# xerial/genome-weaver-align

Hardware: AMD Instinct MI355X
Metric: reads/sec (whole node), 100 bp k≤2 vs hg19, at 1/2/4/8 MI355X (higher is better)
Workload: dtype u64

## Files before the change

genome-weaver-align_amd/csrc/batch_io.hip:

```cpp
#include <hip/hip_runtime.h>

#include <rocprim/device/device_radix_sort.hpp>
#include <rocprim/device/device_scan.hpp>

#include <cstdlib>
#include <stdexcept>
#include <string>

#include "kernels.h"
#include "sam_core.h"
#include "text_core.h"

namespace gwa {

#define FCHK(x)                                                                                         \
  do {                                                                                                  \
    hipError_t e_ = (x);                                                                                \
    if (e_ != hipSuccess) throw std::runtime_error(std::string("sam_format: ") + #x + ": " + hipGetErrorString(e_)); \
  } while (0)


__device__ __forceinline__ uint8_t to3bitDev(unsigned char c) {
  switch (c) {
    case 'A': case 'a': return 0;
// ... 29 lines not shown
    w[i] = r ? (lo >> r) | (hi << (32 - r)) : lo;
  }
}
__global__ void __launch_bounds__(256) encodeLenKernel(const char *__restrict__ seq, const uint64_t *__restrict__ seqB,
                                                       const uint64_t *__restrict__ seqE, uint32_t n, uint32_t *__restrict__ codeLen,
                                                       uint32_t *__restrict__ rowLen, uint32_t *__restrict__ lenSeen) {
  const uint32_t r = blockIdx.x * blockDim.x + threadIdx.x;
  if (r > n) return;
  if (r == n) {
    rowLen[n] = 16;
    return;
  }
  const uint64_t b = seqB[r], e = seqE[r];
  uint32_t spaces = 0;
  for (uint64_t a = b & ~(uint64_t)15; a < e; a += 16) {
    const u32x4 c = loadChunk(seq, a);
    const uint32_t w[4] = {c.x, c.y, c.z, c.w};
#pragma unroll
    for (int i = 0; i < 4; ++i) {
      const uint64_t p = a + 4 * i;
      uint32_t m = bytesEq(w[i], ' ');
      const int64_t lo = (int64_t)b - (int64_t)p, hi = (int64_t)e - (int64_t)p;
      const uint32_t keepLo = lo <= 0 ? 0xFFFFFFFFu : lo >= 4 ? 0u : (0xFFFFFFFFu << (8 * lo));
      const uint32_t keepHi = hi >= 4 ? 0xFFFFFFFFu : hi <= 0 ? 0u : (0xFFFFFFFFu >> (8 * (4 - hi)));
      spaces += __builtin_popcount(m & keepLo & keepHi);
    }
  }
  const uint32_t m = (uint32_t)(e - b) - spaces;
  codeLen[r] = m;
  rowLen[r] = (m + 15) & ~15u;
  lenSeen[m < kLenSeen - 1 ? m : kLenSeen - 1] = 1;
}

__global__ void __launch_bounds__(256) encodeWriteKernel(const char *__restrict__ seq, const uint64_t *__restrict__ seqB,
                                                         const uint64_t *__restrict__ seqE, uint32_t n,
                                                         const uint32_t *__restrict__ codeOff,
                                                         const uint32_t *__restrict__ codeLen,
                                                         uint8_t *__restrict__ codes) {
  const uint32_t r = blockIdx.x * blockDim.x + threadIdx.x;
  if (r >= n) return;
  uint8_t *o = codes + codeOff[r];
  const uint64_t b = seqB[r], e = seqE[r];
  const uint32_t m = codeLen[r], row = codeOff[r + 1] - codeOff[r];
  if (m == e - b) {
    for (uint32_t k = 0; k < row; k += 16) {
      uint32_t w[4];
      load16(seq, b + k, w);
      u32x4 v;
      uint32_t c[4];
#pragma unroll
      for (int i = 0; i < 4; ++i) {
        const int valid = (int)m - (int)(k + 4 * i);
        const uint32_t keep = valid >= 4 ? 0xFFFFFFFFu : valid <= 0 ? 0u : (0xFFFFFFFFu >> (8 * (4 - valid)));
        c[i] = to3bit4(w[i]) & keep;
      }
      v.x = c[0]; v.y = c[1]; v.z = c[2]; v.w = c[3];
      *reinterpret_cast<u32x4 *>(o + k) = v;
    }
    return;
  }
  uint32_t k = 0;
  for (uint64_t i = b; i < e; ++i)
    if (seq[i] != ' ') o[k++] = to3bitDev((unsigned char)seq[i]);
  for (; k < row; ++k) o[k] = 0;
}

void launchEncode(const char *seq, const uint64_t *seqB, const uint64_t *seqE, uint32_t n, uint32_t *codeLen, uint32_t *rowLen,
                  uint32_t *codeOff, uint32_t *lenSeen, uint8_t *codes, void *scanTmp, size_t scanTmpBytes, int pass,
                  hipStream_t s) {
  const dim3 grid((n + 1 + 255) / 256);
  if (pass == 0) {
    hipLaunchKernelGGL(encodeLenKernel, grid, dim3(256), 0, s, seq, seqB, seqE, n, codeLen, rowLen, lenSeen);
    FCHK(hipGetLastError());
    size_t b = scanTmpBytes;
    FCHK(rocprim::exclusive_scan(scanTmp, b, rowLen, codeOff, (uint32_t)0, (size_t)n + 1, rocprim::plus<uint32_t>(), s));
  } else {
    hipLaunchKernelGGL(encodeWriteKernel, grid, dim3(256), 0, s, seq, seqB, seqE, n, codeOff, codeLen, codes);
    FCHK(hipGetLastError());
  }
}

size_t encodeScanTempBytes(uint32_t n) {
  size_t b = 0;
  FCHK(rocprim::exclusive_scan(nullptr, b, (uint32_t *)nullptr, (uint32_t *)nullptr, (uint32_t)0, (size_t)n + 1,
                               rocprim::plus<uint32_t>(), (hipStream_t)0));
  return b;
}

__device__ __forceinline__ bool isWsDev(unsigned char c) { return c == ' ' || (c >= '\t' && c <= '\r') || (c >= 0x1c && c <= 0x1f); }

__device__ __forceinline__ uint64_t lineAt(const char *__restrict__ t, uint64_t len, uint64_t pos, uint64_t *e) {
  if (pos >= len) {
    *e = len;
    return len;
  }
  uint64_t i = pos;
  while (i < len && t[i] != '\n' && t[i] != '\r') ++i;
  *e = i;
  if (i == len) return len;
  if (t[i] == '\r' && i + 1 < len && t[i + 1] == '\n') return i + 2;
  return i + 1;
}

__global__ void __launch_bounds__(256) fastqFieldsKernel(const char *__restrict__ t, uint64_t len, const uint64_t *__restrict__ start,
                                                         uint32_t n, uint64_t *__restrict__ f, uint32_t *__restrict__ err) {
  const uint32_t r = blockIdx.x * blockDim.x + threadIdx.x;
  if (r >= n) return;
  uint64_t he, se, pe, qe;
  const uint64_t hb = start[r];
  const uint64_t sb = lineAt(t, len, hb, &he);
// ... 16 lines not shown
void launchFastqFields(const char *text, uint64_t len, const uint64_t *start, uint32_t n, uint64_t *fields,
                       uint32_t *err, hipStream_t s) {
  if (n == 0) return;
  hipLaunchKernelGGL(fastqFieldsKernel, dim3((n + 255) / 256), dim3(256), 0, s, text, len, start, n, fields, err);
  FCHK(hipGetLastError());
}


__device__ __forceinline__ int samUnit(SamOut &o, const SamText &t, uint32_t r, const OutHeader *oh, const OutHit *hits,
                                       const uint16_t *cig, const PairSpec &ps) {
  if (ps.np) return samPair(o, t, r, ps.np, oh, hits, cig, ps.minIns, ps.maxIns, ps.resc);
  return samRead(o, t, r, oh[r], hits, cig);
}

__global__ void __launch_bounds__(256) samLenKernel(SamText t, const OutHeader *__restrict__ oh, const OutHit *__restrict__ hits,
                                                    const uint16_t *__restrict__ cig, const uint32_t *__restrict__ idx,
                                                    uint32_t first, uint32_t n, uint64_t *__restrict__ len,
                                                    uint32_t *__restrict__ err, PairSpec ps) {
  const uint32_t j = blockIdx.x * blockDim.x + threadIdx.x;
  if (j > n) return;
  if (j == n) {
    len[n] = 0;
    return;
  }
  const uint32_t r = idx ? idx[j] : first + j;
  SamOut o{nullptr, 0};
  if (samUnit(o, t, r, oh, hits, cig, ps) != 0) {
    atomicMin(err, j);
    o.n = 0;
  }
  len[j] = o.n;
}

template <int STAGE>
__global__ void __launch_bounds__(64) samWriteKernel(SamText t, const OutHeader *__restrict__ oh, const OutHit *__restrict__ hits,
                                                     const uint16_t *__restrict__ cig, const uint32_t *__restrict__ idx,
                                                     uint32_t first, uint32_t n, const uint64_t *__restrict__ off,
                                                     char *__restrict__ out, PairSpec ps) {
  __shared__ u32x4 stage[STAGE / 16];
  const uint32_t j0 = blockIdx.x * 64, j = j0 + threadIdx.x;
  const uint32_t jEnd = j0 + 64 < n ? j0 + 64 : n;
  const uint64_t gBeg = off[j0], gEnd = off[jEnd];
  const uint64_t base = gBeg & ~(uint64_t)15;
  if (gEnd - base > (uint64_t)STAGE) {
    if (j < n) {
      SamOut o{out + off[j], 0};
      (void)samUnit(o, t, idx ? idx[j] : first + j, oh, hits, cig, ps);
    }
    return;
  }
  if (j < n) {
    SamOut o{reinterpret_cast<char *>(stage) + (off[j] - base), 0};
    (void)samUnit(o, t, idx ? idx[j] : first + j, oh, hits, cig, ps);
  }
  __syncthreads();
  const uint32_t chunks = (uint32_t)((gEnd - base + 15) >> 4);
  for (uint32_t c = threadIdx.x; c < chunks; c += 64) {
    const uint64_t a = base + 16ull * c;
    if (a >= gBeg && a + 16 <= gEnd) {
      *reinterpret_cast<u32x4 *>(out + a) = stage[c];
    } else {
      const char *sb = reinterpret_cast<const char *>(stage) + 16ull * c;
      for (int i = 0; i < 16; ++i)
        if (a + i >= gBeg && a + i < gEnd) out[a + i] = sb[i];
    }
  }
}

void launchSamFormat(const SamText &t, const OutHeader *oh, const OutHit *hits, const uint16_t *cig, const uint32_t *idx,
                     uint32_t first, uint32_t n, uint64_t *len, uint64_t *off, void *scanTmp, size_t *scanTmpBytes,
                     uint32_t *err, char *out, int pass, hipStream_t s, const PairSpec &ps, uint64_t totalBytes) {
  const dim3 grid((n + 1 + 255) / 256);
  if (pass == 0) {
    hipLaunchKernelGGL(samLenKernel, grid, dim3(256), 0, s, t, oh, hits, cig, idx, first, n, len, err, ps);
    FCHK(hipGetLastError());
  } else if (pass == 1) {
    FCHK(rocprim::exclusive_scan(scanTmp, *scanTmpBytes, len, off, (uint64_t)0, (size_t)n + 1, rocprim::plus<uint64_t>(), s));
  } else {
    if (n == 0) return;
    const dim3 g64((n + 63) / 64);
    const uint64_t need = n ? totalBytes * 64 * 103 / 100 / n + 16 : 0;
    const char *stg = getenv("GWA_SAM_STAGE");
    if (stg && atoi(stg) > 0) {
      if (atoi(stg) <= 1024)
        hipLaunchKernelGGL(samWriteKernel<1024>, g64, dim3(64), 0, s, t, oh, hits, cig, idx, first, n, off, out, ps);
      else
        hipLaunchKernelGGL(samWriteKernel<4096>, g64, dim3(64), 0, s, t, oh, hits, cig, idx, first, n, off, out, ps);
    } else if (ps.np || need > 32768)
      hipLaunchKernelGGL(samWriteKernel<49152>, g64, dim3(64), 0, s, t, oh, hits, cig, idx, first, n, off, out, ps);
    else if (need > 24576)
      hipLaunchKernelGGL(samWriteKernel<32768>, g64, dim3(64), 0, s, t, oh, hits, cig, idx, first, n, off, out, ps);
    else if (need > 20480 || totalBytes == 0)
      hipLaunchKernelGGL(samWriteKernel<24576>, g64, dim3(64), 0, s, t, oh, hits, cig, idx, first, n, off, out, ps);
    else
      hipLaunchKernelGGL(samWriteKernel<20480>, g64, dim3(64), 0, s, t, oh, hits, cig, idx, first, n, off, out, ps);
    FCHK(hipGetLastError());
  }
}

size_t samScanTempBytes(uint32_t n) {
  size_t b = 0;
  FCHK(rocprim::exclusive_scan(nullptr, b, (uint64_t *)nullptr, (uint64_t *)nullptr, (uint64_t)0, (size_t)n + 1,
                               rocprim::plus<uint64_t>(), (hipStream_t)0));
  return b;
}

__global__ void __launch_bounds__(256) statsKernel(const OutHeader *__restrict__ oh, uint32_t n,
                                                   unsigned long long *__restrict__ acc) {
  __shared__ unsigned long long sh[kStatFields];
  if (threadIdx.x < kStatFields) sh[threadIdx.x] = 0;
  __syncthreads();
  unsigned long long v[kStatFields];
  for (int f = 0; f < kStatFields; ++f) v[f] = 0;
  for (uint32_t r = blockIdx.x * blockDim.x + threadIdx.x; r < n; r += gridDim.x * blockDim.x) {
    const OutHeader &h = oh[r];
    v[0] += (unsigned)h.fmSearches;
    v[1] += (unsigned)h.quickSteps;
    v[2] += (unsigned)h.blocks;
    v[3] += (unsigned)h.searchBlocks;
    v[4] += (unsigned)h.kmerLookups;
    v[5] += (unsigned)h.saReads;
    v[6] += (unsigned)h.quickSa;
    v[7] += (unsigned)h.quickShort;
    v[8] += (unsigned)h.searchShort;
    v[9] += (unsigned)h.states;
    v[10] += (unsigned)h.numSW;
    v[11] += (unsigned)h.verifyBytes;
    v[12] += h.status == ST_MAPPED;
// ... 48 lines not shown
```

genome-weaver-align_amd/csrc/gwa_api.cpp:

```cpp
#include "../../include/gwa.h"

#include <hip/hip_runtime.h>

#include <algorithm>
#include <atomic>
#include <cstdio>
#include <cstdlib>
#include <cstring>
#include <fstream>
#include <map>
#include <mutex>
#include <stdexcept>
#include <string>
#include <thread>
#include <unordered_map>
#include <vector>

#include "bsf_core.h"
#include "sf_core.h"
#include "host_index.h"
#include "kernels.h"
#include "sam.h"
#include "sam_core.h"

// ... 217 lines not shown
  }
  ~Scratch() {
    if (!p) return;
    (void)hipStreamSynchronize(s);
    std::lock_guard<std::mutex> g(ix->scratchMu);
    ix->scratchFree.push_back({p, bytes});
  }
};
}

struct gwa_batch {
  gwa_index *ix = nullptr;
  hipStream_t stream = nullptr;
  gwa_config_t cfg{};
  SearchConfig scfg{};
  uint32_t n = 0;
  bool hasQual = false;
  int maxM = 0, kmax = 0, R = 4;
  bool sfWrap = false;
  char *d_seqText = nullptr, *d_nameText = nullptr, *d_qualText = nullptr;
  const uint64_t *d_seqB = nullptr, *d_seqE = nullptr, *d_nameB = nullptr, *d_nameE = nullptr;
  const uint64_t *d_qualB = nullptr, *d_qualE = nullptr;
  uint8_t *d_qualNull = nullptr;
  uint64_t *d_fieldOwn[3] = {nullptr, nullptr, nullptr};
  uint64_t *d_fmtLen = nullptr, *d_fmtOff = nullptr;
  uint32_t *d_fmtIdx = nullptr, *d_fmtErr = nullptr;
  void *d_fmtTmp = nullptr;
  char *d_fmtText = nullptr;
  size_t fmtCap = 0, fmtTmpBytes = 0, fmtTextCap = 0;
  uint64_t fmtBytes = 0;
  bool fmtWhole = false;
  unsigned long long *d_stats = nullptr;
  bool statsDone = false;
  uint32_t *d_row = nullptr, *d_seen = nullptr;
  void *d_encTmp = nullptr;
  size_t encTmpBytes = 0;
  uint8_t *d_codes = nullptr;
  uint32_t *d_off = nullptr, *d_len = nullptr;
  ScanRes *d_sres = nullptr;
  OutHeader *d_oh = nullptr;
  OutHit *d_hits = nullptr;
  uint16_t *d_cig = nullptr;
  uint32_t *d_list[2] = {nullptr, nullptr};
  uint32_t *d_all = nullptr;
  uint32_t *d_count = nullptr;
  uint64_t *d_stair = nullptr;
  uint32_t *d_stairBase = nullptr;
  uint64_t *d_stairBad = nullptr;
  uint32_t hitCap = 4, cigCap = 64;
  uint64_t poolHits = 0, poolCig = 0;
  uint64_t poolUsedH = 0, poolUsedC = 0;
  StairTables st{};
  gwa_batch_stats_t stats{};
  bool ran = false;
  bool headerOnly = false;
  uint32_t pairs = 0;
  int32_t minIns = 0, maxIns = 0;
  RescueOut *d_rescue = nullptr;
  uint32_t *d_heavy = nullptr;
  std::vector<std::pair<uint32_t, int>> deep;
};

static void freeIndexDev(gwa_index *ix) {
  for (int s = 0; s < 2; ++s) {
    if (ix->d_occ[s]) (void)hipFree(ix->d_occ[s]);
    if (ix->d_sa[s]) (void)hipFree(ix->d_sa[s]);
// ... 359 lines not shown
  }
  SearchConfig &sc = b->scfg;
  sc.k = cfg->k; sc.reportType = cfg->report_type; sc.topL = cfg->top_l; sc.numSplit = cfg->num_split;
  sc.matchScore = cfg->match; sc.mismatchPenalty = cfg->mismatch; sc.splitOpenPenalty = cfg->split_open;
  sc.indelEndSkip = cfg->indel_end_skip; sc.bandWidth = cfg->band_width;
  sc.waitQ16 = getenv("GWA_WAITQ16") ? atoi(getenv("GWA_WAITQ16")) : 0;
  sc.refillMin = 1;
  sc.textSearch = (cfg->num_split <= 1 && !getenv("GWA_NO_TEXT")) ? 1 : 0;
  sc.runAheadMax = getenv("GWA_RUNAHEAD") ? atoi(getenv("GWA_RUNAHEAD")) : 4;
  sc.textCache = getenv("GWA_TEXT_CACHE") ? atoi(getenv("GWA_TEXT_CACHE")) : 0;
  b->stream = batchStream();
  return false;
}

static void batchTail(gwa_batch *b, uint64_t seqBytes) {
  const uint32_t n = b->n;
  const gwa_config_t *cfg = &b->cfg;
  hipStream_t s = b->stream;
  const uint64_t codeBound = seqBytes + 16ull * n + 32;
  if (codeBound > 0xFFFFFFFFull) throw std::runtime_error("read batch too large (> 4 GiB of codes): use fewer reads per batch");
  b->d_codes = bAlloc<uint8_t>(codeBound);
  b->d_off = bAlloc<uint32_t>((size_t)n + 1);
  b->d_len = bAlloc<uint32_t>((size_t)n + 1);
  b->d_row = bAlloc<uint32_t>((size_t)n + 1);
  b->d_seen = bAlloc<uint32_t>(kLenSeen);
  b->encTmpBytes = encodeScanTempBytes(n);
  b->d_encTmp = bAlloc<uint8_t>(b->encTmpBytes);
  std::vector<uint32_t> seen(kLenSeen);
  HIPCHK(hipMemsetAsync(b->d_seen, 0, kLenSeen * sizeof(uint32_t), s));
  launchEncode(b->d_seqText, b->d_seqB, b->d_seqE, n, b->d_len, b->d_row, b->d_off, b->d_seen, b->d_codes, b->d_encTmp,
               b->encTmpBytes, 0, s);
  HIPCHK(hipMemcpyAsync(seen.data(), b->d_seen, kLenSeen * sizeof(uint32_t), hipMemcpyDeviceToHost, s));
  HIPCHK(hipStreamSynchronize(s));
  std::vector<int> lens;
  for (uint32_t m = 0; m < kLenSeen; ++m)
    if (seen[m]) {
      b->maxM = (int)m;
      if ((int)m <= kMaxReadLen) lens.push_back((int)m);
    }
  if (b->maxM > kMaxReadLen)
    throw std::runtime_error("read longer than " + std::to_string(kMaxReadLen) + " bp in this batch (" +
                             std::to_string(b->maxM) + " bp): the device path aligns reads of at most " +
                             std::to_string(kMaxReadLen) + " bp");
  b->sfWrap = false;
  for (int m : lens) {
    int k = (cfg->k > 0 && cfg->k < 1) ? (int)floor((double)((float)m * cfg->k)) : (int)cfg->k;
    b->kmax = std::max(b->kmax, k);
    if (m > 0 && k >= 0 && k <= 31 && sfChunksWrap(m, k + 1)) b->sfWrap = true;
  }
  if (b->kmax > 31) throw std::runtime_error("k > 31 is not supported on the device path");
  {
    const bool sfPath = cfg->strategy == 1;
    const int64_t s = sfPath ? 0 : std::max(1, cfg->num_split), T = (s + 1) * s / 2;
    const int64_t M = std::llabs((int64_t)cfg->match), Nn = std::llabs((int64_t)cfg->mismatch);
    const int64_t S = std::llabs((int64_t)cfg->split_open);
    const int64_t bound = M * b->maxM + (M + Nn) * (255 * (s + 1) + T) + S * T;
    const int lim = sfPath ? 31 : 23;
    if ((!sfPath && cfg->num_split > 64) || bound >= (1LL << lim))
      throw std::runtime_error("scoring parameters too large for the device's queue keys (|score| may reach " +
                               std::to_string(bound) + ", limit 2^" + std::to_string(lim) + ")");
  }
  b->R = b->kmax + 1 <= 4 ? 4 : b->kmax + 1 <= 8 ? 8 : b->kmax + 1 <= 16 ? 16 : 32;
  if (b->scfg.waitQ16 <= 0) b->scfg.waitQ16 = b->R >= 8 ? 8 : 14;
  std::vector<uint64_t> tab, bad;
  std::vector<uint32_t> base;
  buildStairTables(lens, std::max(b->kmax, 0), tab, base, bad);
// ... 224 lines not shown
  hipEvent_t e[3] = {nullptr, nullptr, nullptr};
  Events() {
    for (auto &x : e) HIPCHK(hipEventCreate(&x));
  }
  ~Events() {
    for (auto &x : e)
      if (x) (void)hipEventDestroy(x);
  }
};
}

static SamText samText(const gwa_batch *b);

static int qwFor(int m) { return m <= 128 ? 4 : m <= 256 ? 8 : 16; }

int gwa_batch_run(gwa_batch_t *b) {
  try {
    gwa_index *ix = b->ix;
    HIPCHK(hipSetDevice(ix->device));
    hipStream_t s = b->stream;
    memset(&b->stats, 0, sizeof(b->stats));
    if (b->headerOnly) {
      b->ran = true;
      return 0;
    }
    b->ran = b->statsDone = false;
    b->poolUsedH = b->poolUsedC = 0;
    b->deep.clear();
    ReadsView rv{b->d_codes, b->d_off, b->d_len, b->n};
    Scratch scr(ix, s);
    Events ev;
    hipEvent_t e0 = ev.e[0], e1 = ev.e[1], e2 = ev.e[2];
    HIPCHK(hipEventRecord(e2, s));
    launchEncode(b->d_seqText, b->d_seqB, b->d_seqE, b->n, b->d_len, b->d_row, b->d_off, b->d_seen, b->d_codes,
                 b->d_encTmp, b->encTmpBytes, 0, s);
    launchEncode(b->d_seqText, b->d_seqB, b->d_seqE, b->n, b->d_len, b->d_row, b->d_off, b->d_seen, b->d_codes,
                 b->d_encTmp, b->encTmpBytes, 1, s);
    HIPCHK(hipMemsetAsync(b->d_count, 0, 16 * sizeof(uint32_t), s));
    HIPCHK(hipEventRecord(e0, s));
    const bool sf = b->cfg.strategy == 1;
    if (!sf)
      launchQuickscan(qwFor(b->maxM), ix->view, b->scfg, rv, b->d_sres, b->d_oh, outSlots(b), b->d_list[0],
                      b->d_count, s);
    const bool sfSort = sf && b->R >= 8 && !(getenv("GWA_SEARCH_SORT") && atoi(getenv("GWA_SEARCH_SORT")) == 0);
    if (sfSort) launchKeyscan(qwFor(b->maxM), ix->view, b->scfg, rv, b->d_sres, s);
    HIPCHK(hipGetLastError());
    HIPCHK(hipEventRecord(e1, s));
    uint32_t nSearch = b->n;
    if (!sf) HIPCHK(hipMemcpyAsync(&nSearch, b->d_count, 4, hipMemcpyDeviceToHost, s));
    HIPCHK(hipStreamSynchronize(s));
    float qms = 0, ems = 0;
    HIPCHK(hipEventElapsedTime(&qms, e0, e1));
    HIPCHK(hipEventElapsedTime(&ems, e2, e0));
    b->stats.quickscan_ms = qms;
    b->stats.encode_ms = ems;
    double searchMs = 0;
    int cur = 0;
    uint32_t n = nSearch;
    const bool sortLists = !(getenv("GWA_SEARCH_SORT") && atoi(getenv("GWA_SEARCH_SORT")) == 0);
    bool sfSorted = false;
    const int m = std::max(b->maxM, 1);
    int t = 0, regrow = 0, launches = 0;
    int gArena = 0, gHits = 0, gList = 0, gCigar = 0, gCand = 0;
    int arenaMaxLog = 24;
    if (const char *e = getenv("GWA_MAX_STATES_LOG2"))
      arenaMaxLog = std::max(16, std::min(24, atoi(e)));
    const bool hybrid = !sf && b->R >= 8;
    struct ResBuf {
// ... 773 lines not shown
```

genome-weaver-align_amd/csrc/sam_core.h:

```cpp
#pragma once
#include "gwa_layout.h"

namespace gwa {

struct SamText {
  const char *name;
  const uint64_t *nameB, *nameE;
  const char *qual;
  const uint64_t *qualB, *qualE;
  const uint8_t *qualNull;
  const uint8_t *codes;
  const uint32_t *codeOff, *codeLen;
  const char *ctg;
  const uint64_t *ctgOff;
  const int32_t *chrKey;
  int32_t starKey, emptyKey;
};

struct SamOut {
  char *p;
  uint64_t n;
  GWA_HD void ch(char c) {
    if (p) p[n] = c;
    ++n;
  }
  GWA_HD void bytes(const char *s, uint64_t len) {
    if (p) {
      for (uint64_t i = 0; i < len; i += 16) {
        char b[16];
#pragma unroll
        for (int k = 0; k < 16; ++k) b[k] = i + k < len ? s[i + k] : 0;
#pragma unroll
        for (int k = 0; k < 16; ++k)
          if (i + k < len) p[n + i + k] = b[k];
      }
    }
    n += len;
  }
  template <unsigned long L>
  GWA_HD void lit(const char (&s)[L]) {
    bytes(s, L - 1);
  }
  GWA_HD void num(int64_t v) {
    const bool neg = v < 0;
    uint64_t u = neg ? (uint64_t)(-(v + 1)) + 1 : (uint64_t)v;
    uint64_t d0 = 0, d1 = 0, d2 = 0;
    int k = 0;
    do {
      const uint64_t q = u / 10, dig = u - q * 10;
      if (k < 8) d0 |= dig << (8 * k);
      else if (k < 16) d1 |= dig << (8 * (k - 8));
      else d2 |= dig << (8 * (k - 16));
      ++k;
      u = q;
    } while (u);
    if (neg) ch('-');
    for (int i = k - 1; i >= 0; --i) {
      const uint64_t w = i < 8 ? d0 : i < 16 ? d1 : d2;
      ch((char)('0' + (int)((w >> (8 * (i & 7))) & 0xFF)));
    }
  }
};

GWA_HD bool qualAbsent(const SamText &t, uint32_t r) { return t.qual == nullptr || (t.qualNull && t.qualNull[r]); }

namespace samfmt {

constexpr char kSym[5] = {'A', 'C', 'G', 'T', 'N'};
GWA_HD char sym(unsigned x) { return (char)((0x4E54474341ULL >> (8 * x)) & 0xFF); }
constexpr char kOp[8] = {'M', 'I', 'D', 'N', 'S', 'H', 'P', 'X'};

GWA_HD char stateCh(int numHits) { return numHits > 0 ? (numHits == 1 ? 'U' : 'R') : 'N'; }

struct CigSpec {
  const uint16_t *a;
  int na;
  int preS;
  int postS;
  const uint16_t *b;
  int nb;
};

struct CigEmit {
  SamOut &o;
  int pt = -1;
  int64_t pl = 0;
  GWA_HD explicit CigEmit(SamOut &o_) : o(o_) {}
  GWA_HD void flush() {
    if (pt >= 0) {
      o.num(pl);
      o.ch(kOp[pt & 7]);
    }
  }
  GWA_HD void raw(int t, int64_t l) {
    flush();
    pt = t;
    pl = l;
  }
  GWA_HD void add(int t, int64_t l) {
    if (pt == t) pl += l;
    else raw(t, l);
  }
};
// ... 12 lines not shown
  CigSpec cig;
  int seqA, seqB;
  int qualA, qualB;
  int stateHead, stateSelf;
  bool hasSplit;
};

struct Ctx {
  const SamText &t;
  uint32_t r;
  const OutHit *hits;
  int m;
  int strand;
  bool qualNull;
  uint64_t q0, qn;
  bool npe = false;
};

GWA_HD int32_t nameKey(const Ctx &cx, int chr) {
  if (chr >= 0) return cx.t.chrKey[chr];
  if (chr == CHR_STAR) return cx.t.starKey;
  if (chr == CHR_EMPTY) return cx.t.emptyKey;
  return -2147483647 - 1;
}

GWA_HD void chrName(SamOut &o, Ctx &cx, int chr) {
  if (chr >= 0) o.bytes(cx.t.ctg + cx.t.ctgOff[chr], cx.t.ctgOff[chr + 1] - cx.t.ctgOff[chr]);
  else if (chr == CHR_STAR) o.ch('*');
  else if (chr == CHR_EMPTY) {
  } else cx.npe = true;
}

GWA_HD void emitSeq(SamOut &o, const Ctx &cx, int a, int b) {
  const uint8_t *c = cx.t.codes + cx.t.codeOff[cx.r];
  for (int j0 = a; j0 < b; j0 += 16) {
    uint8_t x[16];
#pragma unroll
    for (int k = 0; k < 16; ++k) {
      const int j = j0 + k;
      x[k] = j < b ? (cx.strand == 0 ? c[j] : c[cx.m - 1 - j]) : 0;
    }
#pragma unroll
    for (int k = 0; k < 16; ++k)
      if (j0 + k < b) o.ch(sym(cx.strand == 0 ? x[k] : (x[k] < 4 ? 3 - x[k] : 4)));
  }
}

GWA_HD void emitQual(SamOut &o, const Ctx &cx, int a, int b) {
  if (cx.qualNull) {
    o.ch('*');
    return;
  }
  const char *q = cx.t.qual + cx.q0;
  for (int j0 = a; j0 < b; j0 += 16) {
    char x[16];
#pragma unroll
    for (int k = 0; k < 16; ++k) {
      const int j = j0 + k;
      x[k] = j < b ? (cx.strand == 0 ? q[j] : q[cx.qn - 1 - j]) : 0;
    }
#pragma unroll
    for (int k = 0; k < 16; ++k)
      if (j0 + k < b) o.ch(x[k]);
  }
}

GWA_HD void emitState(SamOut &o, const Ctx &cx, int head, int self) {
  for (int t = head; t >= 0; t = cx.hits[t].next) {
    const char c = stateCh(cx.hits[t].numHits);
    o.ch(t == self ? c : (char)(c - 'A' + 'a'));
  }
}

GWA_HD bool lineOne(SamOut &o, Ctx &cx, const Rec &r, const Rec *split, bool hasSegments, bool isFirst, bool eachMapped) {
  int flag = 0;
  if (hasSegments) flag |= 0x1;
  if (r.strand == 1) flag |= 0x10;
  if (isFirst) {
    flag |= 0x40;
    if (r.numBestHits <= 0 || (split && split->numBestHits <= 0)) eachMapped = false;
  } else if (!split) {
    flag |= 0x80;
  }
  if (eachMapped) flag |= 0x2;
  if (r.numBestHits <= 0) flag |= 0x4;
  if (split && split->numBestHits <= 0) flag |= 0x8;
  o.bytes(cx.t.name + cx.t.nameB[cx.r], cx.t.nameE[cx.r] - cx.t.nameB[cx.r]);
  o.ch('\t');
  o.num(flag);
  o.ch('\t');
  chrName(o, cx, r.chr);
  o.ch('\t');
  o.num(r.start);
  o.lit("\t1\t");
  emitCigar(o, r.cig);
  if (!split) {
    o.lit("\t*\t0\t0");
  } else {
    const int32_t ck = nameKey(cx, r.chr), sk = nameKey(cx, split->chr);
    if (r.chr != CHR_NULL && split->chr != CHR_NULL && ck != cx.t.starKey && ck == sk) {
      o.lit("\t=");
    } else {
      o.ch('\t');
      chrName(o, cx, split->chr);
    }
    o.ch('\t');
    o.num(split->start);
    o.ch('\t');
    o.num((int64_t)split->end - r.start);
  }
  o.ch('\t');
  emitSeq(o, cx, r.seqA, r.seqB);
  o.ch('\t');
  emitQual(o, cx, r.qualA, r.qualB);
  if (r.numBestHits > 0) {
    if (r.nm >= 0) {
      o.lit("\tNM:i:");
      o.num(r.nm);
    }
    o.lit("\tXP:Z:");
// ... 64 lines not shown
          rec.cig.postS = s.matchLength;
          rec.chr = h.chr; rec.strand = h.strand; rec.start = h.pos; rec.end = h.pos + m; rec.nm = h.diff;
          rec.numBestHits = numHits;
          emitRec(o, cx, rec, nullptr, false);
        } else {
          if (s.chr == CHR_NULL) return -1;
          rec.cig.b = cig + s.cigarOff;
          rec.cig.nb = (int)s.cigarLen;
          rec.chr = s.chr; rec.strand = s.strand; rec.start = s.pos - h.matchLength; rec.end = s.pos - h.matchLength + m;
          rec.nm = s.diff; rec.numBestHits = numHits; rec.stateSelf = h.next;
          emitRec(o, cx, rec, nullptr, false);
        }
      } else {
        if (h.chr == CHR_NULL) return -1;
        rec.cig.postS = s.qEnd - s.qStart;
        rec.chr = h.chr; rec.strand = h.strand; rec.start = h.pos; rec.end = h.pos; rec.nm = h.diff;
        rec.numBestHits = numHits;
        emitRec(o, cx, rec, nullptr, false);
      }
    } else {
      if (!sU) return 0;
      if (s.chr == CHR_NULL) return -1;
      rec.cig = CigSpec{nullptr, 0, h.matchLength, -1, cig + s.cigarOff, (int)s.cigarLen};
      rec.chr = s.chr; rec.strand = s.strand; rec.start = s.pos - h.matchLength; rec.end = s.pos - h.matchLength + m;
      rec.nm = s.diff; rec.numBestHits = numHits; rec.stateSelf = h.next;
      emitRec(o, cx, rec, nullptr, false);
    }
  }
  o.ch('\n');
  return cx.npe ? -1 : 0;
}

GWA_HD void samUnmapped(SamOut &o, const SamText &t, uint32_t r) {
  o.bytes(t.name + t.nameB[r], t.nameE[r] - t.nameB[r]);
  o.lit("\t68\t*\t0\t1\t\t*\t0\t0\t");
  const uint8_t *c = t.codes + t.codeOff[r];
  const uint32_t len = t.codeLen[r];
  for (uint32_t j0 = 0; j0 < len; j0 += 16) {
    uint8_t x[16];
#pragma unroll
    for (int k = 0; k < 16; ++k) x[k] = j0 + k < len ? c[j0 + k] : 0;
#pragma unroll
    for (int k = 0; k < 16; ++k)
      if (j0 + k < len) o.ch(samfmt::sym(x[k] > 4 ? 4 : x[k]));
  }
  o.ch('\t');
  if (!qualAbsent(t, r)) o.bytes(t.qual + t.qualB[r], t.qualE[r] - t.qualB[r]);
  else o.ch('*');
  o.ch('\n');
}

GWA_HD int samRead(SamOut &o, const SamText &t, uint32_t r, const OutHeader &h, const OutHit *hits, const uint16_t *cig) {
  if (h.status == ST_UNMAPPED) {
    samUnmapped(o, t, r);
    return 0;
  }
  if (h.status != ST_MAPPED) return -1;
  const OutHit *hb = hits + h.hitOff;
  const uint16_t *cb = cig + h.cigOff;
  int head = 0;
  for (int c = 0; c < h.nChains; ++c) {
    if (samChain(o, t, r, hb, cb, head) != 0) return -1;
    int x = head;
    while (hb[x].next >= 0) x = hb[x].next;
    head = x + 1;
  }
  return 0;
}


GWA_HD int samRefLen(const uint16_t *cig, const OutHit &h) {
  int l = 0;
  for (uint32_t i = 0; i < h.cigarLen; ++i) {
    const int t = cig[h.cigarOff + i] & 7;
    if (t == 0 || t == 7 || t == 2 || t == 6 || t == 3) l += cig[h.cigarOff + i] >> 3;
  }
  return l;
}

GWA_HD void samMateLine(SamOut &o, const SamText &t, uint32_t r, const OutHit *h, const uint16_t *hc, const OutHit *mate,
                        bool first, bool proper, bool leftmost, int64_t tlenAbs, bool sameChr) {
  int flag = 0x1 | (first ? 0x40 : 0x80);
  if (proper) flag |= 0x2;
  if (!h) flag |= 0x4;
  if (!mate) flag |= 0x8;
  if (h && h->strand == 1) flag |= 0x10;
  if (mate && mate->strand == 1) flag |= 0x20;
  o.bytes(t.name + t.nameB[r], t.nameE[r] - t.nameB[r]);
  o.ch('\t');
  o.num(flag);
  o.ch('\t');
  if (h) {
    o.bytes(t.ctg + t.ctgOff[h->chr], t.ctgOff[h->chr + 1] - t.ctgOff[h->chr]);
    o.ch('\t');
    o.num(h->pos);
    o.lit("\t1\t");
    for (uint32_t i = 0; i < h->cigarLen; ++i) {
      o.num(hc[h->cigarOff + i] >> 3);
      o.ch(samfmt::kOp[hc[h->cigarOff + i] & 7]);
    }
    o.ch('\t');
  } else {
    o.lit("*\t0\t1\t*\t");
  }
  if (mate) {
    if (h && sameChr) o.ch('=');
    else o.bytes(t.ctg + t.ctgOff[mate->chr], t.ctgOff[mate->chr + 1] - t.ctgOff[mate->chr]);
    o.ch('\t');
    o.num(mate->pos);
    o.ch('\t');
  } else {
    o.lit("*\t0\t");
  }
  o.num(h && mate && sameChr ? (leftmost ? tlenAbs : -tlenAbs) : 0);
  o.ch('\t');
  const bool rev = h && h->strand == 1;
  const uint8_t *c = t.codes + t.codeOff[r];
  const int m = (int)t.codeLen[r];
  for (int j = 0; j < m; ++j) {
    const uint8_t x = rev ? c[m - 1 - j] : c[j];
    o.ch(samfmt::sym(!rev ? (x > 4 ? 4 : x) : (x < 4 ? 3 - x : 4)));
  }
  o.ch('\t');
  if (qualAbsent(t, r)) {
    o.ch('*');
  } else {
    const uint64_t q0 = t.qualB[r], qn = t.qualE[r] - t.qualB[r];
    for (uint64_t j = 0; j < qn; ++j) o.ch(rev ? t.qual[q0 + qn - 1 - j] : t.qual[q0 + j]);
  }
  if (h) {
    o.lit("\tNM:i:");
    o.num(h->diff);
    o.lit("\tXP:Z:");
    o.ch(h->numHits == 1 ? 'U' : 'R');
    o.lit("\tX0:i:");
    o.num(h->numHits);
  }
  o.ch('\n');
}

struct PairChoice {
  const OutHit *a = nullptr, *b = nullptr, *fa = nullptr, *fb = nullptr;
  const uint16_t *ca = nullptr, *cb = nullptr;
  bool ok = true;
};

GWA_HD bool pairProper(const SamText &t, const OutHit &u, const uint16_t *cu, const OutHit &v, const uint16_t *cv,
                       int32_t minIns, int32_t maxIns) {
  if (t.chrKey[u.chr] != t.chrKey[v.chr] || u.strand == v.strand) return false;
  const OutHit &fw = u.strand == 0 ? u : v, &rv = u.strand == 0 ? v : u;
  const uint16_t *rc = u.strand == 0 ? cv : cu;
  const int64_t fs = fw.pos, re = (int64_t)rv.pos + samRefLen(rc, rv) - 1;
  const int64_t tl = re - fs + 1;
  return !(fs > re || tl < minIns || tl > maxIns);
}

GWA_HD bool pairStatusOk(const OutHeader &A, const OutHeader &B) {
  return (A.status == ST_MAPPED || A.status == ST_UNMAPPED) && (B.status == ST_MAPPED || B.status == ST_UNMAPPED);
}
GWA_HD int pairCandidates(const OutHeader &H, const OutHit *hits, int32_t *first) {
  *first = -1;
// ... 105 lines not shown
```

Baseline: 165.0 million.

## Defer long SAM fields to cooperative LDS copy and widen encode parallelism

SAM output now records long copies (name, sequence, quality, including reverse-complement variants) as descriptors in shared memory. After the per-read formatting pass, the whole workgroup copies and converts them with 16-byte vector loads, using byte permutes for base translation and reversal. The encode write kernel is split across eight lanes per read. A redundant encode length pass is skipped when lengths are already current, and the stage size is now computed at runtime with dynamic LDS. The aim is to cut the serial per-byte writes in each thread, at the cost of atomics, more LDS use, extra synchronisation, and more complex code.

```diff
diff --git a/genome-weaver-align_amd/csrc/batch_io.hip b/genome-weaver-align_amd/csrc/batch_io.hip
--- a/genome-weaver-align_amd/csrc/batch_io.hip
+++ b/genome-weaver-align_amd/csrc/batch_io.hip
@@ -85,18 +85,21 @@
   lenSeen[m < kLenSeen - 1 ? m : kLenSeen - 1] = 1;
 }
 
+constexpr uint32_t kEncLanes = 8;
 __global__ void __launch_bounds__(256) encodeWriteKernel(const char *__restrict__ seq, const uint64_t *__restrict__ seqB,
                                                          const uint64_t *__restrict__ seqE, uint32_t n,
                                                          const uint32_t *__restrict__ codeOff,
                                                          const uint32_t *__restrict__ codeLen,
                                                          uint8_t *__restrict__ codes) {
-  const uint32_t r = blockIdx.x * blockDim.x + threadIdx.x;
+  const uint64_t tid = (uint64_t)blockIdx.x * blockDim.x + threadIdx.x;
+  const uint32_t r = (uint32_t)(tid / kEncLanes), sub = (uint32_t)(tid % kEncLanes);
   if (r >= n) return;
-  uint8_t *o = codes + codeOff[r];
+  const uint32_t o0 = codeOff[r];
+  uint8_t *o = codes + o0;
   const uint64_t b = seqB[r], e = seqE[r];
-  const uint32_t m = codeLen[r], row = codeOff[r + 1] - codeOff[r];
+  const uint32_t m = codeLen[r], row = codeOff[r + 1] - o0;
   if (m == e - b) {
-    for (uint32_t k = 0; k < row; k += 16) {
+    for (uint32_t k = 16 * sub; k < row; k += 16 * kEncLanes) {
       uint32_t w[4];
       load16(seq, b + k, w);
       u32x4 v;
@@ -112,6 +115,7 @@
     }
     return;
   }
+  if (sub != 0) return;
   uint32_t k = 0;
   for (uint64_t i = b; i < e; ++i)
     if (seq[i] != ' ') o[k++] = to3bitDev((unsigned char)seq[i]);
@@ -128,7 +132,9 @@
     size_t b = scanTmpBytes;
     FCHK(rocprim::exclusive_scan(scanTmp, b, rowLen, codeOff, (uint32_t)0, (size_t)n + 1, rocprim::plus<uint32_t>(), s));
   } else {
-    hipLaunchKernelGGL(encodeWriteKernel, grid, dim3(256), 0, s, seq, seqB, seqE, n, codeOff, codeLen, codes);
+    if (n == 0) return;
+    const dim3 g8((unsigned)(((uint64_t)n * kEncLanes + 255) / 256));
+    hipLaunchKernelGGL(encodeWriteKernel, g8, dim3(256), 0, s, seq, seqB, seqE, n, codeOff, codeLen, codes);
     FCHK(hipGetLastError());
   }
 }
@@ -211,35 +217,172 @@
   len[j] = o.n;
 }
 
-template <int STAGE>
-__global__ void __launch_bounds__(64) samWriteKernel(SamText t, const OutHeader *__restrict__ oh, const OutHit *__restrict__ hits,
+
+__device__ __forceinline__ void putBytes(char *q, const uint32_t (&W)[4], uint32_t u, uint32_t k) {
+  while (k > 0) {
+    const uint32_t d = u >> 2;
+    const uint32_t lo = d == 0 ? W[0] : d == 1 ? W[1] : d == 2 ? W[2] : W[3];
+    const uint32_t hi = d == 0 ? W[1] : d == 1 ? W[2] : d == 2 ? W[3] : 0u;
+    const uint32_t v = __builtin_amdgcn_alignbit(hi, lo, (u & 3) * 8);
+    if ((((uint32_t)(uintptr_t)q) & 3) == 0 && k >= 4) {
+      *reinterpret_cast<uint32_t *>(q) = v;
+      q += 4; u += 4; k -= 4;
+    } else {
+      *q = (char)v;
+      q += 1; u += 1; k -= 1;
+    }
+  }
+}
+
+typedef const __attribute__((address_space(1))) char *GlobalText;
+__device__ __forceinline__ void loadText16(const char *p, uint32_t (&w)[4]) {
+  u32x4 v;
+  __builtin_memcpy(&v, (GlobalText)(uintptr_t)p, 16);
+  w[0] = v.x; w[1] = v.y; w[2] = v.z; w[3] = v.w;
+}
+
+__device__ void samSmallCopy(char *dst, const char *src, uint32_t len) {
+  if (len == 0) return;
+  uint32_t w[4];
+  loadText16(src, w);
+  putBytes(dst, w, 0, len);
+}
+
+struct SamSpan {
+  const char *src;
+  uint32_t at, len, kind, head, ni;
+};
+__device__ __forceinline__ SamSpan samSpan(const SamField &f) {
+  SamSpan s;
+  s.src = reinterpret_cast<const char *>((uint64_t)f.srcHi << 32 | f.srcLo);
+  s.at = f.w & 0xFFFFu;
+  s.len = (f.w >> 16) & 0x3FFFu;
+  s.kind = f.w >> 30;
+  s.head = (16u - (s.at & 15u)) & 15u;
+  s.ni = (s.len - s.head) >> 4;
+  return s;
+}
+__device__ __forceinline__ const char *spanSrc(const SamSpan &s, uint32_t i0, uint32_t k) {
+  return s.kind >= SAM_SEQ_RC ? s.src + (s.len - i0 - k) : s.src + i0;
+}
+__device__ __forceinline__ void spanConvert(uint32_t kind, const uint32_t (&w)[4], uint32_t (&W)[4]) {
+  if (kind >= SAM_SEQ_RC) {
+#pragma unroll
+    for (int i = 0; i < 4; ++i) {
+      const uint32_t x = kind == SAM_SEQ_RC ? __builtin_amdgcn_perm(0x4Eu, 0x41434754u, w[3 - i]) : w[3 - i];
+      W[i] = __builtin_bswap32(x);
+    }
+  } else {
+#pragma unroll
+    for (int i = 0; i < 4; ++i)
+      W[i] = kind == SAM_SEQ ? __builtin_amdgcn_perm(0x4Eu, 0x54474341u, w[i]) : w[i];
+  }
+}
+
+__device__ __forceinline__ void samServeFields(const SamField *fields, uint32_t D, char *stage, uint32_t lshift) {
+  const uint32_t L = 1u << lshift, G = blockDim.x >> lshift;
+  const uint32_t sub = threadIdx.x & (L - 1), g = threadIdx.x >> lshift;
+  constexpr int U = 4;
+  for (uint32_t d0 = 0; d0 < D; d0 += G * U) {
+    SamSpan sp[U];
+    uint32_t w[U][4];
+    bool on[U];
+#pragma unroll
+    for (int x = 0; x < U; ++x) {
+      const uint32_t d = d0 + x * G + g;
+      on[x] = false;
+      sp[x].ni = 0;
+      if (d < D) {
+        sp[x] = samSpan(fields[d]);
+        on[x] = sub < sp[x].ni;
+        if (on[x]) loadText16(spanSrc(sp[x], sp[x].head + 16 * sub, 16), w[x]);
+      }
+    }
+#pragma unroll
+    for (int x = 0; x < U; ++x)
+      if (on[x]) {
+        uint32_t W[4];
+        spanConvert(sp[x].kind, w[x], W);
+        u32x4 v;
+        v.x = W[0]; v.y = W[1]; v.z = W[2]; v.w = W[3];
+        *reinterpret_cast<u32x4 *>(stage + sp[x].at + sp[x].head + 16 * sub) = v;
+      }
+#pragma unroll
+    for (int x = 0; x < U; ++x)
+      for (uint32_t c = sub + L; c < sp[x].ni; c += L) {
+        uint32_t w2[4], W[4];
+        loadText16(spanSrc(sp[x], sp[x].head + 16 * c, 16), w2);
+        spanConvert(sp[x].kind, w2, W);
+        u32x4 v;
+        v.x = W[0]; v.y = W[1]; v.z = W[2]; v.w = W[3];
+        *reinterpret_cast<u32x4 *>(stage + sp[x].at + sp[x].head + 16 * c) = v;
+      }
+  }
+  for (uint32_t e0 = 0; e0 < 2 * D; e0 += blockDim.x * U) {
+    SamSpan sp[U];
+    uint32_t w[U][4], i0[U], k[U];
+#pragma unroll
+    for (int x = 0; x < U; ++x) {
+      const uint32_t e = e0 + blockDim.x * x + threadIdx.x;
+      k[x] = 0;
+      if (e < 2 * D) {
+        sp[x] = samSpan(fields[e >> 1]);
+        i0[x] = e & 1 ? sp[x].head + 16 * sp[x].ni : 0;
+        k[x] = e & 1 ? sp[x].len - i0[x] : sp[x].head;
+        if (k[x]) loadText16(spanSrc(sp[x], i0[x], k[x]), w[x]);
+      }
+    }
+#pragma unroll
+    for (int x = 0; x < U; ++x)
+      if (k[x]) {
+        uint32_t W[4];
+        spanConvert(sp[x].kind, w[x], W);
+        putBytes(stage + sp[x].at + i0[x], W, sp[x].kind >= SAM_SEQ_RC ? 16 - k[x] : 0, k[x]);
+      }
+  }
+}
+
+constexpr uint32_t kSamWg = 64;
+
+__global__ void __launch_bounds__(kSamWg) samWriteKernel(SamText t, const OutHeader *__restrict__ oh, const OutHit *__restrict__ hits,
                                                      const uint16_t *__restrict__ cig, const uint32_t *__restrict__ idx,
                                                      uint32_t first, uint32_t n, const uint64_t *__restrict__ off,
-                                                     char *__restrict__ out, PairSpec ps) {
-  __shared__ u32x4 stage[STAGE / 16];
-  const uint32_t j0 = blockIdx.x * 64, j = j0 + threadIdx.x;
-  const uint32_t jEnd = j0 + 64 < n ? j0 + 64 : n;
+                                                     char *__restrict__ out, PairSpec ps, uint32_t stageBytes, uint32_t cap,
+                                                     uint32_t lshift) {
+  extern __shared__ u32x4 samLds[];
+  SamField *fields = reinterpret_cast<SamField *>(samLds);
+  const uint32_t descBytes = (cap * (uint32_t)sizeof(SamField) + 4 + 15) & ~15u;
+  uint32_t *count = reinterpret_cast<uint32_t *>(reinterpret_cast<char *>(samLds) + descBytes - 4);
+  char *stage = reinterpret_cast<char *>(samLds) + descBytes;
+  const uint32_t j0 = blockIdx.x * blockDim.x, j = j0 + threadIdx.x;
+  const uint32_t jEnd = j0 + blockDim.x < n ? j0 + blockDim.x : n;
   const uint64_t gBeg = off[j0], gEnd = off[jEnd];
   const uint64_t base = gBeg & ~(uint64_t)15;
-  if (gEnd - base > (uint64_t)STAGE) {
+  if (gEnd - base > (uint64_t)stageBytes) {
     if (j < n) {
       SamOut o{out + off[j], 0};
       (void)samUnit(o, t, idx ? idx[j] : first + j, oh, hits, cig, ps);
     }
     return;
   }
+  if (threadIdx.x == 0) *count = 0;
+  __syncthreads();
   if (j < n) {
-    SamOut o{reinterpret_cast<char *>(stage) + (off[j] - base), 0};
+    SamOut o{stage + (off[j] - base), 0, SamDefer{fields, count, cap, stage}};
     (void)samUnit(o, t, idx ? idx[j] : first + j, oh, hits, cig, ps);
   }
+  __syncthreads();
+  const uint32_t D = *count < cap ? *count : cap;
+  samServeFields(fields, D, stage, lshift);
   __syncthreads();
   const uint32_t chunks = (uint32_t)((gEnd - base + 15) >> 4);
-  for (uint32_t c = threadIdx.x; c < chunks; c += 64) {
+  const u32x4 *st = reinterpret_cast<const u32x4 *>(stage);
+  for (uint32_t c = threadIdx.x; c < chunks; c += blockDim.x) {
     const uint64_t a = base + 16ull * c;
     if (a >= gBeg && a + 16 <= gEnd) {
-      *reinterpret_cast<u32x4 *>(out + a) = stage[c];
+      *reinterpret_cast<u32x4 *>(out + a) = st[c];
     } else {
-      const char *sb = reinterpret_cast<const char *>(stage) + 16ull * c;
+      const char *sb = stage + 16ull * c;
       for (int i = 0; i < 16; ++i)
         if (a + i >= gBeg && a + i < gEnd) out[a + i] = sb[i];
     }
@@ -257,22 +400,24 @@
     FCHK(rocprim::exclusive_scan(scanTmp, *scanTmpBytes, len, off, (uint64_t)0, (size_t)n + 1, rocprim::plus<uint64_t>(), s));
   } else {
     if (n == 0) return;
-    const dim3 g64((n + 63) / 64);
-    const uint64_t need = n ? totalBytes * 64 * 103 / 100 / n + 16 : 0;
+    const uint32_t wg = kSamWg;
+    const dim3 grid2((n + wg - 1) / wg);
+    const char *dfr = getenv("GWA_SAM_DEFER");
+    const uint32_t lines = ps.np ? 2 : 1, cap = dfr && atoi(dfr) == 0 ? 0 : wg * 3 * lines;
+    const uint32_t descBytes = (cap * (uint32_t)sizeof(SamField) + 4 + 15) & ~15u;
+    const uint64_t stageMax = (65536 - descBytes) & ~255u;
+    uint64_t need = totalBytes ? totalBytes * wg * 103 / 100 / n + 16 : 384 * wg;
+    need = (need + 255) & ~(uint64_t)255;
+    uint32_t stage = (uint32_t)(need < 4096 ? 4096 : need > stageMax ? stageMax : need);
     const char *stg = getenv("GWA_SAM_STAGE");
-    if (stg && atoi(stg) > 0) {
-      if (atoi(stg) <= 1024)
-        hipLaunchKernelGGL(samWriteKernel<1024>, g64, dim3(64), 0, s, t, oh, hits, cig, idx, first, n, off, out, ps);
-      else
-        hipLaunchKernelGGL(samWriteKernel<4096>, g64, dim3(64), 0, s, t, oh, hits, cig, idx, first, n, off, out, ps);
-    } else if (ps.np || need > 32768)
-      hipLaunchKernelGGL(samWriteKernel<49152>, g64, dim3(64), 0, s, t, oh, hits, cig, idx, first, n, off, out, ps);
-    else if (need > 24576)
-      hipLaunchKernelGGL(samWriteKernel<32768>, g64, dim3(64), 0, s, t, oh, hits, cig, idx, first, n, off, out, ps);
-    else if (need > 20480 || totalBytes == 0)
-      hipLaunchKernelGGL(samWriteKernel<24576>, g64, dim3(64), 0, s, t, oh, hits, cig, idx, first, n, off, out, ps);
-    else
-      hipLaunchKernelGGL(samWriteKernel<20480>, g64, dim3(64), 0, s, t, oh, hits, cig, idx, first, n, off, out, ps);
+    if (stg && atoi(stg) > 0) stage = atoi(stg) <= 1024 ? 1024 : 4096;
+    const uint64_t avgLine = totalBytes / n / lines;
+    const uint64_t fieldItems = (avgLine > 64 ? (avgLine - 60) / 2 : 2) / 16;
+    uint32_t lshift = 2;
+    while (lshift < 6 && (1u << lshift) < fieldItems) ++lshift;
+    const uint32_t lds = descBytes + stage;
+    hipLaunchKernelGGL(samWriteKernel, grid2, dim3(wg), lds, s, t, oh, hits, cig, idx, first, n, off, out, ps, stage, cap,
+                       lshift);
     FCHK(hipGetLastError());
   }
 }
diff --git a/genome-weaver-align_amd/csrc/gwa_api.cpp b/genome-weaver-align_amd/csrc/gwa_api.cpp
--- a/genome-weaver-align_amd/csrc/gwa_api.cpp
+++ b/genome-weaver-align_amd/csrc/gwa_api.cpp
@@ -273,6 +273,7 @@
   bool fmtWhole = false;
   unsigned long long *d_stats = nullptr;
   bool statsDone = false;
+  bool lenCurrent = false;
   uint32_t *d_row = nullptr, *d_seen = nullptr;
   void *d_encTmp = nullptr;
   size_t encTmpBytes = 0;
@@ -698,6 +699,7 @@
                b->encTmpBytes, 0, s);
   HIPCHK(hipMemcpyAsync(seen.data(), b->d_seen, kLenSeen * sizeof(uint32_t), hipMemcpyDeviceToHost, s));
   HIPCHK(hipStreamSynchronize(s));
+  b->lenCurrent = true;
   std::vector<int> lens;
   for (uint32_t m = 0; m < kLenSeen; ++m)
     if (seen[m]) {
@@ -988,8 +990,11 @@
     Events ev;
     hipEvent_t e0 = ev.e[0], e1 = ev.e[1], e2 = ev.e[2];
     HIPCHK(hipEventRecord(e2, s));
-    launchEncode(b->d_seqText, b->d_seqB, b->d_seqE, b->n, b->d_len, b->d_row, b->d_off, b->d_seen, b->d_codes,
-                 b->d_encTmp, b->encTmpBytes, 0, s);
+    if (!b->lenCurrent) {
+      launchEncode(b->d_seqText, b->d_seqB, b->d_seqE, b->n, b->d_len, b->d_row, b->d_off, b->d_seen, b->d_codes,
+                   b->d_encTmp, b->encTmpBytes, 0, s);
+      b->lenCurrent = true;
+    }
     launchEncode(b->d_seqText, b->d_seqB, b->d_seqE, b->n, b->d_len, b->d_row, b->d_off, b->d_seen, b->d_codes,
                  b->d_encTmp, b->encTmpBytes, 1, s);
     HIPCHK(hipMemsetAsync(b->d_count, 0, 16 * sizeof(uint32_t), s));
diff --git a/genome-weaver-align_amd/csrc/sam_core.h b/genome-weaver-align_amd/csrc/sam_core.h
--- a/genome-weaver-align_amd/csrc/sam_core.h
+++ b/genome-weaver-align_amd/csrc/sam_core.h
@@ -17,12 +17,50 @@
   int32_t starKey, emptyKey;
 };
 
+enum : uint32_t {
+  SAM_COPY = 0,
+  SAM_SEQ = 1,
+  SAM_SEQ_RC = 2,
+  SAM_REV = 3
+};
+constexpr uint32_t kSamDeferMin = 16;
+constexpr uint32_t kSamDeferMax = 1 << 14;
+struct SamField {
+  uint32_t srcLo, srcHi;
+  uint32_t w;
+};
+struct SamDefer {
+  SamField *f = nullptr;
+  uint32_t *count = nullptr;
+  uint32_t cap = 0;
+  char *stage = nullptr;
+};
+#if defined(__HIP_DEVICE_COMPILE__)
+__device__ void samSmallCopy(char *dst, const char *src, uint32_t len);
+#endif
+
 struct SamOut {
   char *p;
   uint64_t n;
+  SamDefer d{};
   GWA_HD void ch(char c) {
     if (p) p[n] = c;
     ++n;
+  }
+  GWA_HD bool defer(const void *src, uint64_t len, uint32_t kind) {
+#if defined(__HIP_DEVICE_COMPILE__)
+    if (d.f && len > kSamDeferMin && len < kSamDeferMax) {
+      const uint32_t slot = atomicAdd(d.count, 1u);
+      if (slot < d.cap) {
+        const uint64_t a = (uint64_t)src;
+        d.f[slot] = SamField{(uint32_t)a, (uint32_t)(a >> 32),
+                             (uint32_t)(p + n - d.stage) | (uint32_t)len << 16 | kind << 30};
+        n += len;
+        return true;
+      }
+    }
+#endif
+    return false;
   }
   GWA_HD void bytes(const char *s, uint64_t len) {
     if (p) {
@@ -37,6 +75,19 @@
     }
     n += len;
   }
+  GWA_HD void text(const char *s, uint64_t len) {
+    if (defer(s, len, SAM_COPY)) return;
+#if defined(__HIP_DEVICE_COMPILE__)
+    if (p && len <= 16) {
+      samSmallCopy(p + n, s, (uint32_t)len);
+      n += len;
+      return;
+    }
+#endif
+    bytes(s, len);
+  }
+  GWA_HD void seq(const uint8_t *c, int m, int a, int b, bool rc);
+  GWA_HD void qual(const char *q, uint64_t qn, int a, int b, bool rev);
   template <unsigned long L>
   GWA_HD void lit(const char (&s)[L]) {
     bytes(s, L - 1);
@@ -69,6 +120,49 @@
 constexpr char kSym[5] = {'A', 'C', 'G', 'T', 'N'};
 GWA_HD char sym(unsigned x) { return (char)((0x4E54474341ULL >> (8 * x)) & 0xFF); }
 constexpr char kOp[8] = {'M', 'I', 'D', 'N', 'S', 'H', 'P', 'X'};
+}
+
+GWA_HD void SamOut::seq(const uint8_t *c, int m, int a, int b, bool rc) {
+  if (b <= a) return;
+  if (!p) {
+    n += (uint64_t)(b - a);
+    return;
+  }
+  if (defer(rc ? c + (m - b) : c + a, (uint64_t)(b - a), rc ? SAM_SEQ_RC : SAM_SEQ)) return;
+  for (int j0 = a; j0 < b; j0 += 16) {
+    uint8_t x[16];
+#pragma unroll
+    for (int k = 0; k < 16; ++k) {
+      const int j = j0 + k;
+      x[k] = j < b ? (rc ? c[m - 1 - j] : c[j]) : 0;
+    }
+#pragma unroll
+    for (int k = 0; k < 16; ++k)
+      if (j0 + k < b) ch(samfmt::sym(rc ? (x[k] < 4 ? 3 - x[k] : 4) : (x[k] > 4 ? 4 : x[k])));
+  }
+}
+
+GWA_HD void SamOut::qual(const char *q, uint64_t qn, int a, int b, bool rev) {
+  if (b <= a) return;
+  if (!p) {
+    n += (uint64_t)(b - a);
+    return;
+  }
+  if (defer(rev ? q + (qn - (uint64_t)b) : q + a, (uint64_t)(b - a), rev ? SAM_REV : SAM_COPY)) return;
+  for (int j0 = a; j0 < b; j0 += 16) {
+    char x[16];
+#pragma unroll
+    for (int k = 0; k < 16; ++k) {
+      const int j = j0 + k;
+      x[k] = j < b ? (rev ? q[qn - 1 - j] : q[j]) : 0;
+    }
+#pragma unroll
+    for (int k = 0; k < 16; ++k)
+      if (j0 + k < b) ch(x[k]);
+  }
+}
+
+namespace samfmt {
 
 GWA_HD char stateCh(int numHits) { return numHits > 0 ? (numHits == 1 ? 'U' : 'R') : 'N'; }
 
@@ -147,18 +241,7 @@
 }
 
 GWA_HD void emitSeq(SamOut &o, const Ctx &cx, int a, int b) {
-  const uint8_t *c = cx.t.codes + cx.t.codeOff[cx.r];
-  for (int j0 = a; j0 < b; j0 += 16) {
-    uint8_t x[16];
-#pragma unroll
-    for (int k = 0; k < 16; ++k) {
-      const int j = j0 + k;
-      x[k] = j < b ? (cx.strand == 0 ? c[j] : c[cx.m - 1 - j]) : 0;
-    }
-#pragma unroll
-    for (int k = 0; k < 16; ++k)
-      if (j0 + k < b) o.ch(sym(cx.strand == 0 ? x[k] : (x[k] < 4 ? 3 - x[k] : 4)));
-  }
+  o.seq(cx.t.codes + cx.t.codeOff[cx.r], cx.m, a, b, cx.strand != 0);
 }
 
 GWA_HD void emitQual(SamOut &o, const Ctx &cx, int a, int b) {
@@ -166,18 +249,7 @@
     o.ch('*');
     return;
   }
-  const char *q = cx.t.qual + cx.q0;
-  for (int j0 = a; j0 < b; j0 += 16) {
-    char x[16];
-#pragma unroll
-    for (int k = 0; k < 16; ++k) {
-      const int j = j0 + k;
-      x[k] = j < b ? (cx.strand == 0 ? q[j] : q[cx.qn - 1 - j]) : 0;
-    }
-#pragma unroll
-    for (int k = 0; k < 16; ++k)
-      if (j0 + k < b) o.ch(x[k]);
-  }
+  o.qual(cx.t.qual + cx.q0, cx.qn, a, b, cx.strand != 0);
 }
 
 GWA_HD void emitState(SamOut &o, const Ctx &cx, int head, int self) {
@@ -200,7 +272,7 @@
   if (eachMapped) flag |= 0x2;
   if (r.numBestHits <= 0) flag |= 0x4;
   if (split && split->numBestHits <= 0) flag |= 0x8;
-  o.bytes(cx.t.name + cx.t.nameB[cx.r], cx.t.nameE[cx.r] - cx.t.nameB[cx.r]);
+  o.text(cx.t.name + cx.t.nameB[cx.r], cx.t.nameE[cx.r] - cx.t.nameB[cx.r]);
   o.ch('\t');
   o.num(flag);
   o.ch('\t');
@@ -331,20 +403,11 @@
 }
 
 GWA_HD void samUnmapped(SamOut &o, const SamText &t, uint32_t r) {
-  o.bytes(t.name + t.nameB[r], t.nameE[r] - t.nameB[r]);
+  o.text(t.name + t.nameB[r], t.nameE[r] - t.nameB[r]);
   o.lit("\t68\t*\t0\t1\t\t*\t0\t0\t");
-  const uint8_t *c = t.codes + t.codeOff[r];
-  const uint32_t len = t.codeLen[r];
-  for (uint32_t j0 = 0; j0 < len; j0 += 16) {
-    uint8_t x[16];
-#pragma unroll
-    for (int k = 0; k < 16; ++k) x[k] = j0 + k < len ? c[j0 + k] : 0;
-#pragma unroll
-    for (int k = 0; k < 16; ++k)
-      if (j0 + k < len) o.ch(samfmt::sym(x[k] > 4 ? 4 : x[k]));
-  }
-  o.ch('\t');
-  if (!qualAbsent(t, r)) o.bytes(t.qual + t.qualB[r], t.qualE[r] - t.qualB[r]);
+  o.seq(t.codes + t.codeOff[r], (int)t.codeLen[r], 0, (int)t.codeLen[r], false);
+  o.ch('\t');
+  if (!qualAbsent(t, r)) o.text(t.qual + t.qualB[r], t.qualE[r] - t.qualB[r]);
   else o.ch('*');
   o.ch('\n');
 }
@@ -385,7 +448,7 @@
   if (!mate) flag |= 0x8;
   if (h && h->strand == 1) flag |= 0x10;
   if (mate && mate->strand == 1) flag |= 0x20;
-  o.bytes(t.name + t.nameB[r], t.nameE[r] - t.nameB[r]);
+  o.text(t.name + t.nameB[r], t.nameE[r] - t.nameB[r]);
   o.ch('\t');
   o.num(flag);
   o.ch('\t');
@@ -414,18 +477,14 @@
   o.num(h && mate && sameChr ? (leftmost ? tlenAbs : -tlenAbs) : 0);
   o.ch('\t');
   const bool rev = h && h->strand == 1;
-  const uint8_t *c = t.codes + t.codeOff[r];
   const int m = (int)t.codeLen[r];
-  for (int j = 0; j < m; ++j) {
-    const uint8_t x = rev ? c[m - 1 - j] : c[j];
-    o.ch(samfmt::sym(!rev ? (x > 4 ? 4 : x) : (x < 4 ? 3 - x : 4)));
-  }
+  o.seq(t.codes + t.codeOff[r], m, 0, m, rev);
   o.ch('\t');
   if (qualAbsent(t, r)) {
     o.ch('*');
   } else {
-    const uint64_t q0 = t.qualB[r], qn = t.qualE[r] - t.qualB[r];
-    for (uint64_t j = 0; j < qn; ++j) o.ch(rev ? t.qual[q0 + qn - 1 - j] : t.qual[q0 + j]);
+    const uint64_t qn = t.qualE[r] - t.qualB[r];
+    o.qual(t.qual + t.qualB[r], qn, 0, (int)qn, rev);
   }
   if (h) {
     o.lit("\tNM:i:");
```

After: 170.3 million, median of 6. 1.03x the previous value.
